# happykygo/GNN-eCommerce

Hardware: AMD Instinct MI355X
Metric: edges propagated/sec per LGConv layer (higher is better)
Workload: dtype f32; 1 GPU; configs[1]: 1639358 users x 54571 items, 20314816 directed edges, 3 LGConv layers, emb_dim 64, get_embedding (K hops + fused layer sum); parallelism=single, seed=0

## Files before the change

gnn-ecommerce_amd/_native.py:

```python
from __future__ import annotations

import ctypes
import os
from ctypes import CFUNCTYPE, POINTER, Structure, c_char_p, c_float, c_int, c_int32, c_int64, c_size_t, c_uint64, c_void_p
from typing import Optional

import torch

LIB_NAME = "liblgconv_hip.so"
LIB_PATH = os.environ.get("LGCN_LIB_PATH") or os.path.join(os.path.dirname(os.path.abspath(__file__)), "csrc", LIB_NAME)
ABI_VERSION = 14

ST_INDEX_OOB = 1
ST_SAMPLER_EXHAUSTED = 2

class SweepCfg(Structure):
    _fields_ = [("n_bands", c_int32), ("waves_per_band_round", c_int32), ("row_cap", c_int32), ("piece_cap", c_int32),
                ("lookahead", c_int32), ("groups", c_int32), ("round_order", c_int32), ("light_len", c_int32)]


class SweepDims(Structure):
    _fields_ = [("n_bands", c_int32), ("rounds", c_int32), ("row_cap", c_int32), ("piece_cap", c_int32),
                ("n_rows", c_int32), ("groups", c_int32),
                ("n_waves", c_int64), ("n_slabs", c_int64), ("n_slots", c_int64), ("n_entries", c_int64),
# ... 111 lines not shown
                              c_void_p, c_void_p, c_void_p]),
    "lgc_fold_in": (c_int, [c_void_p, c_void_p, c_void_p, c_int64, c_void_p, c_void_p, c_int64, c_int64, c_void_p, c_void_p,
                            c_int64, c_int64, c_float, c_int32, c_int32, c_void_p, c_int64, c_void_p, c_void_p]),
    "lgc_score_rows": (c_int, [c_void_p, c_int64, c_int64, c_void_p, c_int64, c_void_p, c_int64, c_int32, c_int32, c_void_p,
                               c_int64, c_void_p, c_void_p]),
    "lgc_topk_hits": (c_int, [c_void_p, c_int64, c_int32, c_void_p, c_void_p, c_void_p, c_int64, c_int64, c_void_p, c_void_p,
                              c_void_p, c_void_p]),
    "lgc_metric_sums": (c_int, [c_void_p, c_void_p, c_int64, c_void_p, c_void_p, c_void_p]),
    "lgc_rank_metrics": (c_int, [c_void_p, c_int64, c_int32, c_void_p, c_void_p, c_void_p, c_void_p, c_int64, c_int64,
                                 POINTER(c_int32), c_int32, c_void_p, c_void_p, c_void_p, c_void_p, c_void_p]),
    "lgc_column_sums": (c_int, [c_void_p, c_int64, c_int64, c_int32, c_void_p, c_void_p]),
    "lgc_topk_coverage": (c_int, [c_void_p, c_int64, c_int32, c_int64, POINTER(c_int32), c_int32, c_int64, c_void_p, c_void_p,
                                  c_void_p, c_void_p]),
    "lgc_bfs_init": (c_int, [c_void_p, c_int32, c_int64, c_void_p, c_void_p, c_void_p, c_void_p]),
    "lgc_bfs_level": (c_int, [c_void_p, c_void_p, c_int32, c_int32, c_int32, c_void_p, c_int32, c_uint64, c_void_p, c_void_p,
                              c_void_p, c_void_p, c_void_p]),
    "lgc_bfs_resolve": (c_int, [c_void_p, c_void_p, c_int32, c_int64, c_int64, c_void_p, c_int32, c_void_p, c_void_p, c_void_p,
                                c_void_p]),
    "lgc_bfs_backtrack": (c_int, [c_void_p, c_void_p, c_int64, c_void_p, c_int32, c_void_p, c_void_p, c_int32, c_int64,
                                  c_void_p, c_int32, c_void_p]),
    "lgc_sample_triples": (c_int, [c_void_p, c_int64, c_void_p, c_void_p, c_void_p, c_void_p, c_int64, c_int64, c_uint64,
                                   c_uint64, c_void_p, c_void_p, c_void_p, c_void_p]),
    "lgc_pair_dot": (c_int, [c_void_p, c_int64, c_int32, c_int64, c_void_p, c_void_p, c_int64, c_void_p,
                             c_void_p, c_void_p]),
    "lgc_reduce_workspace_bytes": (c_size_t, [c_int64, c_int64]),
    "lgc_reduce_count": (c_int, [c_void_p, c_void_p, c_int64, c_int64, c_int64, c_int32, c_void_p, c_size_t, c_void_p, c_void_p,
                                 c_void_p]),
    "lgc_reduce_fill": (c_int, [c_void_p, c_void_p, c_int64, c_int64, c_int64, c_void_p, c_void_p, c_int64, c_int64, c_void_p,
                                c_void_p, c_void_p]),
    "lgc_reduce_gram_workspace_bytes": (c_size_t, [c_int64]),
    "lgc_reduce_gram_count": (c_int, [c_void_p, c_void_p, c_int64, c_int64, c_int64, c_void_p, c_int64, c_void_p, c_size_t,
                                      c_void_p, c_void_p]),
    "lgc_reduce_gram_fill": (c_int, [c_void_p, c_int64, c_int64, c_int64, c_int64, c_void_p, c_void_p, c_void_p]),
    "lgc_attribute": (c_int, [POINTER(AttrArgsC), c_void_p]),
    "lgc_row_rnorm": (c_int, [c_void_p, c_int64, c_int64, c_int32, c_void_p, c_void_p]),
    "lgc_item_neighbors_workspace_bytes": (c_size_t, [c_int64, c_int64, c_int32, c_int32]),
    "lgc_item_neighbors": (c_int, [c_void_p, c_int64, c_int64, c_int32, c_void_p, c_int64, c_void_p, c_void_p, c_int32, c_int32,
                                   c_int32, c_void_p, c_void_p, c_void_p, c_size_t, c_void_p, c_void_p]),
    "lgc_rerank_route": (c_int, [c_int32, c_int32]),
    "lgc_rerank_mmr": (c_int, [c_void_p, c_int64, c_int64, c_int32, c_void_p, c_void_p, c_int64, c_void_p, c_int64, c_int64,
                               c_int32, c_int32, c_float, c_void_p, c_void_p, c_void_p, c_void_p, c_void_p]),
    "lgc_list_diversity": (c_int, [c_void_p, c_int64, c_int64, c_int32, c_void_p, c_void_p, c_int64, c_int64, c_int32,
                                   POINTER(c_int32), c_int32, c_void_p, c_int64, c_void_p, c_void_p]),
}


class NativeLibraryError(RuntimeError):
    """The HIP library is missing, stale, or a call into it failed."""


_lib: Optional[ctypes.CDLL] = None


def load() -> ctypes.CDLL:
    global _lib
    if _lib is not None:
        return _lib
    if not os.path.isfile(LIB_PATH):
        raise NativeLibraryError(
            f"{LIB_PATH} not found: the MI355X propagation library has not been built. "
            "Run `python -c 'import __graft_entry__ as g; g.build()'` (or `make -C gnn-ecommerce_amd/csrc`). "
            "There is no CPU or PyTorch fallback for this path.")
    try:
        lib = ctypes.CDLL(LIB_PATH)
    except OSError as exc:
        raise NativeLibraryError(f"cannot load {LIB_PATH}: {exc}") from exc
# ... 71 lines not shown
```

gnn-ecommerce_amd/csrc/lgconv_reduce.hip:

```cpp
#include "lgconv_common.h"

#include <hipcub/hipcub.hpp>

namespace {

inline size_t r_align_up(size_t v, size_t a) { return (v + a - 1) / a * a; }

struct ReduceWs {
    int32_t *incount;
    int32_t *keep_scan;
    int32_t *ent_scan;
    long long *pair_scan;
    void *cub;
    size_t cub_bytes;
};

size_t reduce_ws(void *base, int64_t n_nodes, int64_t n_edges, ReduceWs *ws) {
    size_t cb32 = 0, cb64 = 0;
    int32_t *n32 = nullptr;
    long long *n64 = nullptr;
    const int64_t longest = std::max<int64_t>(n_edges, n_nodes) + 1;
    (void)hipcub::DeviceScan::ExclusiveSum(nullptr, cb32, n32, n32, (int)longest, (hipStream_t)0);
    (void)hipcub::DeviceScan::ExclusiveSum(nullptr, cb64, n64, n64, (int)longest, (hipStream_t)0);
    const size_t cb = std::max(cb32, cb64);
// ... 17 lines not shown
    unsigned long long *keys_in, *keys_out;
    double *vals_in, *vals_out;
    int32_t *head_scan;
    void *cub;
    size_t cub_bytes;
};

size_t gram_ws(void *base, int64_t n_pairs, GramWs *ws) {
    size_t cb_sort = 0, cb_scan = 0;
    unsigned long long *nk = nullptr;
    double *nv = nullptr;
    int32_t *n32 = nullptr;
    const int64_t n = std::max<int64_t>(n_pairs, 1);
    (void)hipcub::DeviceRadixSort::SortPairs(nullptr, cb_sort, nk, nk, nv, nv, (int)n, 0, 64, (hipStream_t)0);
    (void)hipcub::DeviceScan::ExclusiveSum(nullptr, cb_scan, n32, n32, (int)(n + 1), (hipStream_t)0);
    const size_t cb = std::max(cb_sort, cb_scan);
    const uintptr_t p = reinterpret_cast<uintptr_t>(base);
    size_t off = 0;
    auto take = [&](size_t bytes) { const size_t at = off; off += r_align_up(bytes, 256); return p + at; };
    const uintptr_t a_ki = take((size_t)n * 8), a_ko = take((size_t)n * 8), a_vi = take((size_t)n * 8), a_vo = take((size_t)n * 8),
                    a_hs = take((size_t)(n + 1) * 4), a_cub = take(cb);
    if (ws) {
        ws->keys_in = reinterpret_cast<unsigned long long *>(a_ki);
        ws->keys_out = reinterpret_cast<unsigned long long *>(a_ko);
        ws->vals_in = reinterpret_cast<double *>(a_vi);
        ws->vals_out = reinterpret_cast<double *>(a_vo);
        ws->head_scan = reinterpret_cast<int32_t *>(a_hs);
        ws->cub = reinterpret_cast<void *>(a_cub);
        ws->cub_bytes = cb;
    }
    return off + 256;
}

__device__ inline int32_t row_of_entry(const int32_t *__restrict__ rowptr, int32_t n_rows, int32_t e) {
    int32_t lo = 0, hi = n_rows;
    while (hi - lo > 1) {
        const int32_t mid = lo + (hi - lo) / 2;
        if (rowptr[mid] <= e) lo = mid; else hi = mid;
    }
    return lo;
}

__global__ void k_reduce_incount(const int32_t *__restrict__ rowptr, const lgc_entry *__restrict__ entries, int32_t n_nodes,
                                 int32_t split, int32_t n_edges, int32_t *__restrict__ incount) {
    const int32_t e_begin = max(rowptr[split], 0), e_end = min(rowptr[n_nodes], n_edges);
    for (int64_t e = e_begin + (int64_t)blockIdx.x * blockDim.x + threadIdx.x; e < e_end; e += (int64_t)gridDim.x * blockDim.x) {
        const int32_t c = entries[e].col;
        if (c >= 0 && c < split) atomicAdd(incount + c, 1);
    }
}

__global__ void k_reduce_keep(const int32_t *__restrict__ rowptr, const int32_t *__restrict__ incount, int32_t split,
                              int32_t max_deg, int32_t *__restrict__ keep) {
    const int64_t u = (int64_t)blockIdx.x * blockDim.x + threadIdx.x;
    if (u > split) return;
    int32_t k = 0;
    if (u < split) k = (rowptr[u + 1] - rowptr[u] <= max_deg && incount[u] <= max_deg) ? 0 : 1;
    keep[u] = k;
}

__global__ void k_reduce_user_map(const int32_t *__restrict__ keep_scan, int32_t split, int32_t *__restrict__ user_map) {
    const int64_t u = (int64_t)blockIdx.x * blockDim.x + threadIdx.x;
    if (u >= split) return;
    user_map[u] = keep_scan[u + 1] != keep_scan[u] ? keep_scan[u] : -1;
}

__global__ void k_reduce_entry_flags(const int32_t *__restrict__ rowptr, const lgc_entry *__restrict__ entries, int32_t n_nodes,
// ... 93 lines not shown
__global__ void k_gram_fill_entries(const unsigned long long *__restrict__ keys, const double *__restrict__ vals,
                                    const int32_t *__restrict__ head_scan, long long n_pairs, int32_t n_h, int32_t n_out,
                                    lgc_entry *__restrict__ out) {
    const int64_t p = (int64_t)blockIdx.x * blockDim.x + threadIdx.x;
    if (p >= n_pairs) return;
    const int32_t dst = head_scan[p];
    if (head_scan[p + 1] == dst || dst < 0 || dst >= n_out) return;
    const unsigned long long key = keys[p];
    double sum = 0.0;
    for (int64_t q = p; q < n_pairs && keys[q] == key; ++q) sum += vals[q];
    lgc_entry en;
    en.col = n_h + (int32_t)(uint32_t)(key & 0xFFFFFFFFull);
    en.val = (float)sum;
    out[dst] = en;
}

__global__ void k_gram_fill_rowptr(const unsigned long long *__restrict__ keys, const int32_t *__restrict__ head_scan,
                                   long long n_pairs, int32_t n_h, int32_t n_items, int32_t *__restrict__ rowptr_out) {
    const int64_t r = (int64_t)blockIdx.x * blockDim.x + threadIdx.x;
    if (r > (int64_t)n_h + n_items) return;
    if (r <= n_h) {
        rowptr_out[r] = 0;
        return;
    }
    const unsigned long long want = (unsigned long long)(uint32_t)(r - n_h) << 32;
    long long lo = 0, hi = n_pairs;
    while (lo < hi) {
        const long long mid = lo + (hi - lo) / 2;
        if (keys[mid] < want) lo = mid + 1; else hi = mid;
    }
    rowptr_out[r] = head_scan[lo];
}

int reduce_args_ok(const int32_t *rowptr, const lgc_entry *entries, int64_t n_nodes, int64_t n_edges, int64_t split) {
    if (n_nodes < 0 || n_edges < 0 || split < 0) return LGC_E_INVAL;
    if (n_nodes >= INT32_MAX || n_edges >= INT32_MAX) return LGC_E_RANGE;
    if (!rowptr || split <= 0 || split >= n_nodes || (n_edges > 0 && !entries)) return LGC_E_INVAL;
    return 0;
}

}

extern "C" {

size_t lgc_reduce_workspace_bytes(int64_t n_nodes, int64_t n_edges) {
    if (n_nodes < 0 || n_edges < 0 || n_nodes >= INT32_MAX || n_edges >= INT32_MAX) return 0;
    return reduce_ws(nullptr, n_nodes, n_edges, nullptr);
}

int lgc_reduce_count(const int32_t *rowptr, const lgc_entry *entries, int64_t n_nodes, int64_t n_edges, int64_t split,
                     int32_t max_deg, void *workspace, size_t workspace_bytes, int32_t *user_map, int64_t *totals,
                     void *stream_) {
    if (const int rc = reduce_args_ok(rowptr, entries, n_nodes, n_edges, split)) return rc;
    if (max_deg < 0 || !workspace || !user_map || !totals) return LGC_E_INVAL;
    if (workspace_bytes < lgc_reduce_workspace_bytes(n_nodes, n_edges)) return LGC_E_WORKSPACE;
    if (reinterpret_cast<uintptr_t>(workspace) % 256 != 0) return LGC_E_ALIGN;
    hipStream_t st = as_stream(stream_);
    ReduceWs ws;
    reduce_ws(workspace, n_nodes, n_edges, &ws);
    const int32_t n = (int32_t)n_nodes, sp = (int32_t)split;
    hipError_t err = hipMemsetAsync(ws.incount, 0, (size_t)(split + 1) * 4, st);
    if (err != hipSuccess) return (int)err;
    if (n_edges > 0)
        hipLaunchKernelGGL(k_reduce_incount, dim3((unsigned)std::min<int64_t>(ceil_div(n_edges, kBlock), 256 * 16)), dim3(kBlock), 0,
                           st, rowptr, entries, n, sp, (int32_t)n_edges, ws.incount);
    hipLaunchKernelGGL(k_reduce_keep, dim3(ceil_div(split + 1, kBlock)), dim3(kBlock), 0, st, rowptr, ws.incount, sp, max_deg,
// ... 60 lines not shown
    hipLaunchKernelGGL(k_gram_expand, dim3(ceil_div(n_edges, kBlock)), dim3(kBlock), 0, st, rowptr, entries, n, sp, ws.pair_scan,
                       (long long)n_pairs, (int32_t)n_edges, gw.keys_in, gw.vals_in);
    err = hipcub::DeviceRadixSort::SortPairs(gw.cub, gw.cub_bytes, gw.keys_in, gw.keys_out, gw.vals_in, gw.vals_out, (int)n_pairs,
                                             0, 64, st);
    if (err != hipSuccess) return (int)err;
    hipLaunchKernelGGL(k_gram_heads, dim3(ceil_div(n_pairs + 1, kBlock)), dim3(kBlock), 0, st, gw.keys_out, (long long)n_pairs,
                       gw.head_scan);
    err = hipcub::DeviceScan::ExclusiveSum(gw.cub, gw.cub_bytes, gw.head_scan, gw.head_scan, (int)(n_pairs + 1), st);
    if (err != hipSuccess) return (int)err;
    err = hipMemcpyAsync(total, gw.head_scan + n_pairs, sizeof(int32_t), hipMemcpyDeviceToDevice, st);
    if (err != hipSuccess) return (int)err;
    return (int)hipGetLastError();
}

int lgc_reduce_gram_fill(const void *gram_workspace, int64_t n_pairs, int64_t n_kept, int64_t n_items, int64_t n_out,
                         int32_t *rowptr_out, lgc_entry *entries_out, void *stream_) {
    if (n_pairs < 0 || n_kept < 0 || n_items < 1 || n_out < 0 || !rowptr_out) return LGC_E_INVAL;
    if (n_pairs >= INT32_MAX || n_kept + n_items >= INT32_MAX) return LGC_E_RANGE;
    if (n_out > n_pairs || (n_pairs > 0 && !gram_workspace) || (n_out > 0 && !entries_out)) return LGC_E_INVAL;
    if (reinterpret_cast<uintptr_t>(gram_workspace) % 256 != 0) return LGC_E_ALIGN;
    hipStream_t st = as_stream(stream_);
    const int64_t rows = n_kept + n_items;
    if (n_pairs == 0) return (int)hipMemsetAsync(rowptr_out, 0, (size_t)(rows + 1) * 4, st);
    GramWs gw;
    gram_ws(const_cast<void *>(gram_workspace), n_pairs, &gw);
    hipLaunchKernelGGL(k_gram_fill_rowptr, dim3(ceil_div(rows + 1, kBlock)), dim3(kBlock), 0, st, gw.keys_out, gw.head_scan,
                       (long long)n_pairs, (int32_t)n_kept, (int32_t)n_items, rowptr_out);
    if (n_out > 0)
        hipLaunchKernelGGL(k_gram_fill_entries, dim3(ceil_div(n_pairs, kBlock)), dim3(kBlock), 0, st, gw.keys_out, gw.vals_out,
                           gw.head_scan, (long long)n_pairs, (int32_t)n_kept, (int32_t)n_out, entries_out);
    return (int)hipGetLastError();
}

}
```

gnn-ecommerce_amd/graph.py:

```python
from __future__ import annotations

import os
from collections import OrderedDict
from dataclasses import dataclass, field
from typing import Dict, List, Optional, Tuple

import torch
from torch import Tensor

from . import _native

SHORT_MAX = int(os.environ.get("LGCN_SHORT_MAX", "32"))
CHUNK_LEN = int(os.environ.get("LGCN_CHUNK_LEN", "256"))
USER_CHUNK_LEN = int(os.environ.get("LGCN_USER_CHUNK_LEN", "4096"))
TILE_WIDTHS = (8, 16, 32)
USE_TILES = os.environ.get("LGCN_TILES", "1") == "1"
TILES_PER_WAVE = int(os.environ.get("LGCN_TILES_PER_WAVE", "1"))
TILE_ORDER = os.environ.get("LGCN_TILE_ORDER", "cold")
USE_SWEEP = os.environ.get("LGCN_SWEEP", "auto")
SWEEP_MIN_ENTRIES = int(os.environ.get("LGCN_SWEEP_MIN_ENTRIES", "1000000"))
SWEEP_ADAPTIVE_BANDS = os.environ.get("LGCN_SWEEP_ADAPTIVE_BANDS", "1") == "1"
SWEEP_PIECE_ENTRIES = int(os.environ.get("LGCN_SWEEP_PIECE_ENTRIES", "20"))
SWEEP_CFG = dict(n_bands=int(os.environ.get("LGCN_SWEEP_BANDS", "8")), waves_per_band_round=int(os.environ.get("LGCN_SWEEP_WAVES", "256")),
                 row_cap=int(os.environ.get("LGCN_SWEEP_ROW_CAP", "78")),
                 piece_cap=int(os.environ.get("LGCN_SWEEP_PIECE_CAP", "64")),
                 lookahead=int(os.environ.get("LGCN_SWEEP_LOOKAHEAD", "64")),
                 groups=4,
                 round_order=int(os.environ.get("LGCN_SWEEP_ROUND_ORDER", "2")))
SWEEP_WIDE = os.environ.get("LGCN_SWEEP_WIDE", "1") == "1"
SWEEP_LIGHT_LEN = os.environ.get("LGCN_SWEEP_LIGHT_LEN", "auto")
SWEEP_LIGHT_LEN_WIDE = os.environ.get("LGCN_SWEEP_LIGHT_LEN_WIDE", "0")


def _light_len(value: str) -> int:
    return -1 if value == "auto" else max(int(value), 0)


PLAN_TIMING = os.environ.get("LGCN_PLAN_TIMING", "0") == "1"
# ... 625 lines not shown
    i32 = dict(dtype=torch.int32, device=dev)
    ws_bytes = lib.lgc_reduce_workspace_bytes(num_nodes, n_edges)
    ws = torch.empty(max(ws_bytes, 1), **u8)
    user_map = torch.empty(max(split, 1), **i32)
    totals = torch.empty(4, dtype=torch.int64, device=dev)
    args = (_native.ptr(rowptr), _native.ptr(entries), num_nodes, n_edges, split)
    with torch.cuda.device(dev):
        st = _native.stream_of(dev)
        _native.check(lib.lgc_reduce_count(*args, int(max_deg), _native.ptr(ws), ws_bytes, _native.ptr(user_map),
                                           _native.ptr(totals), st), "lgc_reduce_count")
        n_h, user_nnz, nnz, n_pairs = totals.tolist()
        rowptr_h = torch.empty(n_h + n_items + 1, **i32)
        entries_h = torch.empty((nnz, 2), **i32)
        _native.check(lib.lgc_reduce_fill(*args, _native.ptr(ws), _native.ptr(user_map), n_h, nnz, _native.ptr(rowptr_h),
                                          _native.ptr(entries_h) if nnz else None, st), "lgc_reduce_fill")
        gws_bytes = lib.lgc_reduce_gram_workspace_bytes(n_pairs)
        if gws_bytes == 0:
            return None
        gws = torch.empty(gws_bytes, **u8)
        total = torch.empty(1, dtype=torch.int64, device=dev)
        code = lib.lgc_reduce_gram_count(*args, _native.ptr(ws), n_pairs, _native.ptr(gws), gws_bytes, _native.ptr(total), st)
        if code == -4:
            return None
        _native.check(code, "lgc_reduce_gram_count")
        gram_nnz = int(total.item())
        gram_rowptr = torch.empty(n_h + n_items + 1, **i32)
        gram_entries = torch.empty((gram_nnz, 2), **i32)
        _native.check(lib.lgc_reduce_gram_fill(_native.ptr(gws), n_pairs, n_h, n_items, gram_nnz, _native.ptr(gram_rowptr),
                                               _native.ptr(gram_entries) if gram_nnz else None, st), "lgc_reduce_gram_fill")
    return ReducedCSR(int(max_deg), n_h, n_items, user_map[:split], rowptr_h, entries_h, user_nnz, n_pairs, gram_rowptr,
                      gram_entries)


@dataclass
class ReducedGraph:
    csr: ReducedCSR
    n_h: int
    offset: int
    user_op_h: Optional[Operator]
    item_op_h: Optional[Operator]
    gram_op: Optional[Operator]

    def nbytes(self) -> int:
        c = self.csr
        total = sum(t.numel() * 4 for t in (c.user_map, c.rowptr, c.entries, c.gram_rowptr, c.gram_entries))
        for op in (self.user_op_h, self.item_op_h, self.gram_op):
            if op is not None:
                total += op.plan.chunks.numel() * 4 + sum(tc.slab.numel() * 4 + tc.order.numel() * 4 + tc.meta.numel() * 4
                                                          for tc in (op._tiles or []))
                total += sum(sw.nbytes() for sw in op._sweep.values())
        return total


def sweep_choice(lib, dim: int, table_rows: int, stride: int) -> int:
    sweep = int(lib.lgc_sweep_ok(dim, table_rows, stride))
    return 0 if (sweep == 2 and not SWEEP_WIDE) else sweep


def _check_table(t: Tensor, name: str) -> None:
    _native.require_device(t, name)
    if t.dtype != torch.float32 or t.dim() != 2 or t.stride(1) != 1:
        raise TypeError(f"{name} must be a 2-D fp32 tensor with unit inner stride, got {t.dtype} {tuple(t.shape)}")


class PropGraph:

    def __init__(self, edge_index: Tensor, edge_weight: Optional[Tensor], num_nodes: int,
                 normalize: bool = True, short_max: int = SHORT_MAX, chunk_len: int = CHUNK_LEN,
                 keep_edge_values: bool = False):
        _native.require_device(edge_index, "edge_index")
        if edge_index.dtype != torch.int64 or edge_index.dim() != 2 or edge_index.size(0) != 2:
            raise TypeError("edge_index must be an int64 tensor of shape [2, E]")
        if edge_weight is not None:
            _native.require_device(edge_weight, "edge_weight")
            if edge_weight.dtype != torch.float32 or edge_weight.shape != (edge_index.size(1),):
                raise TypeError("edge_weight must be fp32 of shape [E]")
            if edge_weight.device != edge_index.device:
                raise RuntimeError("edge_index and edge_weight must be on the same device")
        self.device = edge_index.device
# ... 73 lines not shown
        auto = forced is None and ELIMINATE_MAX_DEG == "auto"
        max_deg = int(forced) if forced is not None else (ELIMINATE_AUTO_MAX_DEG if auto else int(ELIMINATE_MAX_DEG))
        if max_deg <= 0:
            return None
        key = ("reduced", max_deg, auto)
        if key in self._halves:
            return self._halves[key]
        got = None
        if not auto or self.halves(False)[1].sweep_cols is not None:
            got = self._build_reduced(max_deg)
            if got is not None and auto:
                removed = self.forward_op.nnz - got.csr.nnz
                if got.csr.gram_nnz > ELIMINATE_MAX_GRAM_SHARE * removed:
                    got = None
        self._halves[key] = got
        return got

    def _build_reduced(self, max_deg: int) -> Optional[ReducedGraph]:
        op = self.forward_op
        csr = build_reduced_csr(op.rowptr, op.entries, self.split, self.num_nodes, max_deg)
        if csr is None:
            return None
        n_h, n_rows = csr.n_h, csr.n_h + csr.n_items
        user_chunk = max(self.chunk_len, USER_CHUNK_LEN)
        user_op_h = item_op_h = gram_op = None
        if n_h > 0:
            user_op_h = Operator.build(n_rows, csr.rowptr, csr.entries, 0, n_h, self.short_max, user_chunk,
                                       sweep_cols=(n_h, n_rows))
        if csr.nnz - csr.user_nnz > 0:
            item_op_h = Operator.build(n_rows, csr.rowptr, csr.entries, n_h, n_rows, self.short_max, self.chunk_len,
                                       sweep_cols=(0, n_h))
        if csr.gram_nnz > 0:
            gram_op = Operator.build(n_rows, csr.gram_rowptr, csr.gram_entries, n_h, n_rows, self.short_max, GRAM_CHUNK_LEN)
        return ReducedGraph(csr, n_h, self.split - n_h, user_op_h, item_op_h, gram_op)

    def prepare(self, dim: int, table_rows: Optional[int] = None, transpose: bool = False) -> "PropGraph":
        lib = _native.load()
        rows = self.num_nodes if table_rows is None else int(table_rows)
        stride = dim if dim % 32 == 0 else (dim + 31) // 32 * 32
        ops = self.halves(transpose) if self.split is not None else ((self.transpose_op if transpose else self.forward_op),)
        ops = [(op, rows) for op in ops]
        red = self.reduced(transpose)
        if red is not None:
            ops += [(op, max(rows - red.offset, 0)) for op in (red.user_op_h, red.item_op_h, red.gram_op) if op is not None]
        import time
        for op, rows in ops:
            t0 = time.perf_counter()
            if op.tiled and dim >= 4:
                op.tiles
            if PLAN_TIMING:
                torch.cuda.synchronize(self.device)
                print(f"[plan] rows [{op.plan.row_begin}, {op.plan.row_end}): tile classes {time.perf_counter() - t0:.3f} s", flush=True)
            t0 = time.perf_counter()
            if op.sweep_cols is not None:
                groups = sweep_choice(lib, dim, rows, stride)
                if groups:
                    op.sweep_plan(groups)
            if PLAN_TIMING:
                torch.cuda.synchronize(self.device)
                print(f"[plan] rows [{op.plan.row_begin}, {op.plan.row_end}): sweep plan total {time.perf_counter() - t0:.3f} s", flush=True)
        torch.cuda.synchronize(self.device)
        return self

    @property
    def transpose_op(self) -> Operator:
        if self._transpose_op is None:
            if self._edge_index is None:
                raise _native.NativeLibraryError("this graph was loaded from a file without its COO: the transposed "
                                                 "operator (backward pass) needs a graph built from edge_index")
            self._transpose_op = self._build(by_source=True)
        return self._transpose_op

    def save(self, path: str, extra: Optional[Dict[str, Tensor]] = None, meta: Optional[Dict[str, str]] = None) -> None:
        from safetensors.torch import save_file
        op = self.forward_op
        tensors = {"rowptr": op.rowptr, "entries": op.entries, "deg": self.deg, "dis": self.dis}
        for k, v in (extra or {}).items():
# ... 113 lines not shown
```

gnn-ecommerce_amd/propagate.py:

```python
from __future__ import annotations

import os
from typing import List, Optional, Sequence

import torch
from torch import Tensor
from torch.autograd.function import once_differentiable

from . import _native
from .graph import Operator, PropGraph, apply_rows


HOP_EVENT_LOG: Optional[list] = None


def _timed_apply(op: Operator, x: Tensor, out: Tensor, **kw) -> None:
    if HOP_EVENT_LOG is None:
        op.apply(x, out, **kw)
        return
    start, end = torch.cuda.Event(enable_timing=True), torch.cuda.Event(enable_timing=True)
    start.record()
    op.apply(x, out, **kw)
    end.record()
    HOP_EVENT_LOG.append((start, end))
# ... 23 lines not shown
        h = nxt
    return h


USE_BIPARTITE = os.environ.get("LGCN_BIPARTITE", "1") == "1"

class _HopSpan:

    def __enter__(self):
        self.log = HOP_EVENT_LOG
        if self.log is not None:
            self.start, self.end = torch.cuda.Event(enable_timing=True), torch.cuda.Event(enable_timing=True)
            self.start.record()
        return self

    def __exit__(self, *exc):
        if self.log is not None:
            self.end.record()
            self.log.append((self.start, self.end))


def bipartite_sum(user_op: Operator, item_op: Operator, split: int, x0: Tensor, alphas: Sequence[float],
                  final_rows: Optional[Tensor] = None, reduced=None) -> Tensor:
    k = len(alphas) - 1
    if k == 0:
        return x0 * alphas[0]
    x0 = x0.contiguous()
    n = x0.size(0)
    tables = [x0]
    red = reduced if k >= 2 else None
    rows_items_only = final_rows is not None and SCORED_ITEM_ROWS_ONLY and item_op.listed_rows_pay(final_rows.numel()) \
        if red is not None else False

    def user_step(layer: int, x: Tensor, out_t: Tensor) -> None:
        if red is None or (rows_items_only and layer == k - 1):
            user_op.apply(x, out_t)
        elif red.user_op_h is not None:
            red.user_op_h.apply(x[red.offset:], out_t[red.offset:])

    def item_step(layer: int, out_t: Tensor, a: float = 1.0, r: Optional[Tensor] = None) -> None:
        o = red.offset
        y = out_t[o:]
        have = r is not None
        if red.gram_op is not None:
            red.gram_op.apply(tables[layer - 2][o:], y, a=a, r=r[o:] if have else None, b=1.0 if have else 0.0)
        elif have:
            _native.lincomb(out_t[split:], [(1.0, r[split:])])
        else:
            out_t[split:].zero_()
        if red.item_op_h is not None:
            red.item_op_h.apply(tables[layer - 1][o:], y, a=a, r=y, b=1.0)
    uniform = UNIFORM_ALPHA_SHORTCUT and all(a == alphas[0] for a in alphas) and (UNIFORM_ALPHA_SHORTCUT == "force" or x0.size(1) % 32 == 0)
    for layer in range(1, k + 1):
        with _HopSpan():
            nxt = scratch_table(x0)
            if layer < k:
                if red is None or layer == 1:
                    item_op.apply(tables[-1], nxt)
                else:
                    item_step(layer, nxt)
                user_step(layer, tables[-1], nxt)
                tables.append(nxt)
            else:
                out = torch.empty_like(x0)
                rows_only = final_rows is not None
                if rows_only and SCORED_ITEM_ROWS_ONLY and item_op.listed_rows_pay(final_rows.numel()):
                    mix = nxt
                    _native.lincomb(mix[split:], [(alphas[l], tables[l - 1][split:]) for l in range(1, k + 1)])
                    if all(a == alphas[0] for a in alphas):
                        rest = mix
                    else:
                        rest = scratch_table(x0)
                        _native.lincomb(rest[split:], [(alphas[l], tables[l][split:]) for l in range(0, k)])
# ... 1083 lines not shown
```

include/lgconv_hip.h:

```cpp
#ifndef LGCONV_HIP_H
#define LGCONV_HIP_H

#include <stddef.h>
#include <stdint.h>

#ifdef __cplusplus
extern "C" {
#endif

#define LGC_ABI_VERSION 14

#define LGC_E_INVAL      (-1)
#define LGC_E_DIM        (-2)
#define LGC_E_WORKSPACE  (-3)
#define LGC_E_RANGE      (-4)
#define LGC_E_ALIGN      (-5)

#define LGC_ST_INDEX_OOB 1

typedef struct lgc_entry {
    int32_t col;
    float   val;
} lgc_entry;

// ... 250 lines not shown
#define LGC_BFS_UNSET (-3)
int lgc_bfs_init(const int64_t *sources, int32_t n_sources, int64_t n_nodes, uint64_t *seen, uint64_t *frontier,
                 int32_t *status, void *stream);
int lgc_bfs_level(const int32_t *rowptr, const lgc_entry *entries, int32_t row_begin, int32_t row_end, int32_t short_max,
                  const lgc_chunk *chunks, int32_t n_chunks, uint64_t active, const uint64_t *frontier_in,
                  uint64_t *frontier_out, uint64_t *seen, uint64_t *counters, void *stream);
int lgc_bfs_resolve(const int64_t *sources, const int64_t *targets, int32_t n_sources, int64_t n_targets, int64_t n_nodes,
                    const uint64_t *frontier, int32_t level, int32_t *dist, uint64_t *counters, int32_t *status,
                    void *stream);
int lgc_bfs_backtrack(const int32_t *rowptr, const lgc_entry *entries, int64_t n_nodes, const uint64_t *levels,
                      int32_t n_levels, const int64_t *targets, const int32_t *dist, int32_t n_sources, int64_t n_targets,
                      int64_t *paths, int32_t path_len, void *stream);

#define LGC_ST_SAMPLER_EXHAUSTED 2
int lgc_sample_triples(const int64_t *users, int64_t n,
                       const int32_t *pos_ptr, const int64_t *pos_items,
                       const int32_t *ign_ptr, const int64_t *ign_items,
                       int64_t n_users, int64_t n_items, uint64_t seed, uint64_t step,
                       int64_t *pos_out, int64_t *neg_out, int32_t *status, void *stream);

size_t lgc_reduce_workspace_bytes(int64_t n_nodes, int64_t n_edges);
int lgc_reduce_count(const int32_t *rowptr, const lgc_entry *entries, int64_t n_nodes, int64_t n_edges, int64_t split,
                     int32_t max_deg, void *workspace, size_t workspace_bytes, int32_t *user_map, int64_t *totals,
                     void *stream);
int lgc_reduce_fill(const int32_t *rowptr, const lgc_entry *entries, int64_t n_nodes, int64_t n_edges, int64_t split,
                    const void *workspace, const int32_t *user_map, int64_t n_kept, int64_t n_out, int32_t *rowptr_out,
                    lgc_entry *entries_out, void *stream);
size_t lgc_reduce_gram_workspace_bytes(int64_t n_pairs);
int lgc_reduce_gram_count(const int32_t *rowptr, const lgc_entry *entries, int64_t n_nodes, int64_t n_edges, int64_t split,
                          const void *workspace, int64_t n_pairs, void *gram_workspace, size_t gram_workspace_bytes,
                          int64_t *total, void *stream);
int lgc_reduce_gram_fill(const void *gram_workspace, int64_t n_pairs, int64_t n_kept, int64_t n_items, int64_t n_out,
                         int32_t *rowptr_out, lgc_entry *entries_out, void *stream);

#define LGC_ATTR_MAX_TARGETS 64
#define LGC_ATTR_MAX_TOP 8
typedef struct lgc_attr_args {
    const int64_t   *list_ptr, *list_items;
    const float     *list_weight, *item_dis;
    const int32_t   *rowptr;
    const lgc_entry *entries;
    const int64_t   *row_ids;
    int64_t          n_graph_rows, col_base;
    int64_t          n_rows;
    const float     *fold, *items;
    int64_t          fold_stride, item_stride, n_items;
    const int64_t   *init_rows;
    const float     *init;
    int64_t          init_stride, n_init_rows;
    const int64_t   *targets;
    int64_t          target_stride;
    const int64_t   *contrib_ptr;
    float           *contrib, *base, *total;
    int32_t         *top_pos;
    int64_t         *top_item;
    float           *top_value;
    int32_t         *status;
    float            a0;
    int32_t          normalize, n_targets, top_m, dim;
} lgc_attr_args;

int lgc_attribute(const lgc_attr_args *args, void *stream);

#define LGC_NEIGHBORS_MAX_K 64
int lgc_row_rnorm(const float *table, int64_t stride, int64_t n_rows, int32_t dim, float *out, void *stream);
size_t lgc_item_neighbors_workspace_bytes(int64_t n_queries, int64_t n_items, int32_t k, int32_t slices);
// ... 22 lines not shown
```

Baseline: 40.61 billion edges/s.

## Concatenate reduced user graph and item gram into one banded CSR operator

Builds a combined CSR in which the kept-user rows, an identity block stored in gap rows interleaved between user bands, the item-to-user edges and the item gram entries all live in one matrix. The item step then becomes a single sweep operator call instead of separate gram and item operators with an intermediate write. This removes one pass over the output table per layer and one kernel launch. In exchange it adds padded gap rows and a larger entry array, extra build time, and complex index arithmetic in the layout whose correctness depends on the band mapping matching the sweep configuration.

```diff
diff --git a/gnn-ecommerce_amd/_native.py b/gnn-ecommerce_amd/_native.py
--- a/gnn-ecommerce_amd/_native.py
+++ b/gnn-ecommerce_amd/_native.py
@@ -167,6 +167,11 @@
     "lgc_reduce_gram_count": (c_int, [c_void_p, c_void_p, c_int64, c_int64, c_int64, c_void_p, c_int64, c_void_p, c_size_t,
                                       c_void_p, c_void_p]),
     "lgc_reduce_gram_fill": (c_int, [c_void_p, c_int64, c_int64, c_int64, c_int64, c_void_p, c_void_p, c_void_p]),
+    "lgc_reduce_concat_rows": (c_int64, [c_int64, c_int64, c_int32]),
+    "lgc_reduce_concat": (c_int, [c_void_p, c_void_p, c_int64, c_void_p, c_void_p, c_int64, c_int64, c_int64, c_int32, c_void_p,
+                                  c_void_p, c_void_p, c_void_p, c_int64, c_void_p]),
+    "lgc_reduce_concat_host": (c_int, [c_void_p, c_void_p, c_int64, c_void_p, c_void_p, c_int64, c_int64, c_int64, c_int32,
+                                       c_void_p, c_void_p, c_void_p, c_void_p, c_int64]),
     "lgc_attribute": (c_int, [POINTER(AttrArgsC), c_void_p]),
     "lgc_row_rnorm": (c_int, [c_void_p, c_int64, c_int64, c_int32, c_void_p, c_void_p]),
     "lgc_item_neighbors_workspace_bytes": (c_size_t, [c_int64, c_int64, c_int32, c_int32]),
diff --git a/gnn-ecommerce_amd/csrc/lgconv_reduce.hip b/gnn-ecommerce_amd/csrc/lgconv_reduce.hip
--- a/gnn-ecommerce_amd/csrc/lgconv_reduce.hip
+++ b/gnn-ecommerce_amd/csrc/lgconv_reduce.hip
@@ -73,7 +73,7 @@
     return off + 256;
 }
 
-__device__ inline int32_t row_of_entry(const int32_t *__restrict__ rowptr, int32_t n_rows, int32_t e) {
+__host__ __device__ inline int32_t row_of_entry(const int32_t *__restrict__ rowptr, int32_t n_rows, int32_t e) {
     int32_t lo = 0, hi = n_rows;
     while (hi - lo > 1) {
         const int32_t mid = lo + (hi - lo) / 2;
@@ -233,6 +233,126 @@
     rowptr_out[r] = head_scan[lo];
 }
 
+struct Concat {
+    const int32_t *rp;
+    const lgc_entry *ent;
+    const int32_t *grp;
+    const lgc_entry *gent;
+    int32_t n_kept, n_items, n_gaps, gap_rows, n_phys, n_gram, n_out;
+    int32_t *pos, *gap_start, *rowptr_out;
+    lgc_entry *out;
+};
+
+__host__ __device__ inline int32_t cc_band(const Concat &c, int32_t h) {
+    const int64_t ne = c.rp[c.n_kept];
+    if (ne <= 0) return 0;
+    const int64_t b = (int64_t)c.rp[h] * c.n_gaps / ne;
+    return (int32_t)(b < c.n_gaps - 1 ? b : c.n_gaps - 1);
+}
+
+__host__ __device__ inline int32_t cc_users_upto(const Concat &c, int32_t b) {
+    const int64_t ne = c.rp[c.n_kept];
+    if (b >= c.n_gaps - 1 || ne <= 0) return c.n_kept;
+    int32_t lo = 0, hi = c.n_kept;
+    while (lo < hi) {
+        const int32_t mid = lo + (hi - lo) / 2;
+        if ((int64_t)c.rp[mid] * c.n_gaps < ne * (b + 1)) lo = mid + 1; else hi = mid;
+    }
+    return lo;
+}
+
+__host__ __device__ inline int32_t cc_min(int64_t a, int64_t b) { return (int32_t)(a < b ? a : b); }
+
+__host__ __device__ inline void cc_layout_at(const Concat &c, int64_t t) {
+    if (t < c.n_kept) c.pos[t] = (int32_t)t + c.gap_rows * cc_band(c, (int32_t)t);
+    else if (t < (int64_t)c.n_kept + c.n_gaps) {
+        const int32_t b = (int32_t)(t - c.n_kept);
+        c.gap_start[b] = cc_users_upto(c, b) + c.gap_rows * b;
+    }
+}
+
+__host__ __device__ inline void cc_rowptr_at(const Concat &c, int64_t r) {
+    if (r > (int64_t)c.n_phys + c.n_items) return;
+    int64_t v;
+    if (r >= c.n_phys) {
+        const int32_t i = (int32_t)(r - c.n_phys);
+        v = (int64_t)c.rp[c.n_kept] + c.n_items + (c.rp[c.n_kept + i] - c.rp[c.n_kept]) + c.grp[c.n_kept + i];
+    } else {
+        int32_t before = 0;
+        while (before < c.n_gaps && c.gap_start[before] <= r) ++before;
+        if (before > 0 && r < (int64_t)c.gap_start[before - 1] + c.gap_rows) {
+            const int32_t b = before - 1;
+            const int64_t j = (int64_t)b * c.gap_rows + (r - c.gap_start[b]);
+            v = (int64_t)c.rp[c.gap_start[b] - c.gap_rows * b] + cc_min(j, c.n_items);
+        } else {
+            const int32_t h = (int32_t)(r - (int64_t)c.gap_rows * before);
+            v = (int64_t)c.rp[h] + cc_min((int64_t)before * c.gap_rows, c.n_items);
+        }
+    }
+    c.rowptr_out[r] = (int32_t)v;
+}
+
+__host__ __device__ inline void cc_entry_at(const Concat &c, int64_t t) {
+    const int64_t n_user = c.rp[c.n_kept], n_all = c.rp[c.n_kept + c.n_items];
+    const int64_t first_item_entry = n_user + c.n_items;
+    int64_t dst;
+    lgc_entry en;
+    if (t < n_user) {
+        const int32_t h = row_of_entry(c.rp, c.n_kept, (int32_t)t);
+        en = c.ent[t];
+        en.col = c.n_phys + (en.col - c.n_kept);
+        dst = t + cc_min((int64_t)cc_band(c, h) * c.gap_rows, c.n_items);
+    } else if ((t -= n_user) < c.n_items) {
+        const int32_t b = (int32_t)(t / c.gap_rows);
+        en.col = c.n_phys + (int32_t)t;
+        en.val = 1.0f;
+        dst = (int64_t)c.rp[c.gap_start[b] - c.gap_rows * b] + t;
+    } else if ((t -= c.n_items) < n_all - n_user) {
+        const int64_t e = n_user + t;
+        const int32_t i = row_of_entry(c.rp + c.n_kept, c.n_items, (int32_t)e);
+        en = c.ent[e];
+        en.col = c.pos[en.col];
+        dst = first_item_entry + t + c.grp[c.n_kept + i];
+    } else if ((t -= n_all - n_user) < c.n_gram) {
+        const int32_t i = row_of_entry(c.grp + c.n_kept, c.n_items, (int32_t)t);
+        en = c.gent[t];
+        const int32_t j = en.col - c.n_kept;
+        en.col = c.gap_start[j / c.gap_rows] + j % c.gap_rows;
+        dst = first_item_entry + (c.rp[c.n_kept + i + 1] - n_user) + t;
+    } else {
+        return;
+    }
+    if (dst >= 0 && dst < c.n_out) c.out[dst] = en;
+}
+
+__global__ void k_concat_layout(Concat c) {
+    const int64_t t = (int64_t)blockIdx.x * blockDim.x + threadIdx.x;
+    cc_layout_at(c, t);
+}
+__global__ void k_concat_rowptr(Concat c) {
+    const int64_t r = (int64_t)blockIdx.x * blockDim.x + threadIdx.x;
+    cc_rowptr_at(c, r);
+}
+__global__ void k_concat_entries(Concat c) {
+    const int64_t t = (int64_t)blockIdx.x * blockDim.x + threadIdx.x;
+    if (t < c.n_out) cc_entry_at(c, t);
+}
+
+int concat_args(const int32_t *rowptr, const lgc_entry *entries, int64_t n_entries, const int32_t *gram_rowptr,
+                const lgc_entry *gram_entries, int64_t n_gram, int64_t n_kept, int64_t n_items, int32_t n_gaps,
+                int32_t *user_pos, int32_t *gap_start, int32_t *rowptr_out, lgc_entry *entries_out, int64_t n_out, Concat *c) {
+    if (n_entries < 0 || n_gram < 0 || n_kept < 0 || n_items < 1 || n_gaps < 1 || n_out < 0) return LGC_E_INVAL;
+    if (n_gaps > LGC_REDUCE_MAX_GAPS) return LGC_E_RANGE;
+    const int64_t gap_rows = (n_items + n_gaps - 1) / n_gaps, n_phys = n_kept + gap_rows * n_gaps;
+    if (n_phys + n_items >= INT32_MAX || n_entries + n_items + n_gram >= INT32_MAX) return LGC_E_RANGE;
+    if (!rowptr || !gram_rowptr || !gap_start || !rowptr_out || !entries_out || (n_entries > 0 && !entries) ||
+        (n_gram > 0 && !gram_entries) || (n_kept > 0 && !user_pos) || n_out != n_entries + n_items + n_gram)
+        return LGC_E_INVAL;
+    *c = Concat{rowptr, entries, gram_rowptr, gram_entries, (int32_t)n_kept, (int32_t)n_items, n_gaps, (int32_t)gap_rows,
+                (int32_t)n_phys, (int32_t)n_gram, (int32_t)n_out, user_pos, gap_start, rowptr_out, entries_out};
+    return 0;
+}
+
 int reduce_args_ok(const int32_t *rowptr, const lgc_entry *entries, int64_t n_nodes, int64_t n_edges, int64_t split) {
     if (n_nodes < 0 || n_edges < 0 || split < 0) return LGC_E_INVAL;
     if (n_nodes >= INT32_MAX || n_edges >= INT32_MAX) return LGC_E_RANGE;
@@ -359,4 +479,38 @@
     return (int)hipGetLastError();
 }
 
-}
+int64_t lgc_reduce_concat_rows(int64_t n_kept, int64_t n_items, int32_t n_gaps) {
+    if (n_kept < 0 || n_items < 1 || n_gaps < 1 || n_gaps > LGC_REDUCE_MAX_GAPS) return -1;
+    return n_kept + (n_items + n_gaps - 1) / n_gaps * n_gaps;
+}
+
+int lgc_reduce_concat(const int32_t *rowptr, const lgc_entry *entries, int64_t n_entries, const int32_t *gram_rowptr,
+                      const lgc_entry *gram_entries, int64_t n_gram, int64_t n_kept, int64_t n_items, int32_t n_gaps,
+                      int32_t *user_pos, int32_t *gap_start, int32_t *rowptr_out, lgc_entry *entries_out, int64_t n_out,
+                      void *stream_) {
+    Concat c;
+    if (const int rc = concat_args(rowptr, entries, n_entries, gram_rowptr, gram_entries, n_gram, n_kept, n_items, n_gaps,
+                                   user_pos, gap_start, rowptr_out, entries_out, n_out, &c))
+        return rc;
+    hipStream_t st = as_stream(stream_);
+    hipLaunchKernelGGL(k_concat_layout, dim3(ceil_div(n_kept + n_gaps, kBlock)), dim3(kBlock), 0, st, c);
+    hipLaunchKernelGGL(k_concat_rowptr, dim3(ceil_div((int64_t)c.n_phys + n_items + 1, kBlock)), dim3(kBlock), 0, st, c);
+    hipLaunchKernelGGL(k_concat_entries, dim3(ceil_div(n_out, kBlock)), dim3(kBlock), 0, st, c);
+    return (int)hipGetLastError();
+}
+
+int lgc_reduce_concat_host(const int32_t *rowptr, const lgc_entry *entries, int64_t n_entries, const int32_t *gram_rowptr,
+                           const lgc_entry *gram_entries, int64_t n_gram, int64_t n_kept, int64_t n_items, int32_t n_gaps,
+                           int32_t *user_pos, int32_t *gap_start, int32_t *rowptr_out, lgc_entry *entries_out, int64_t n_out) {
+    Concat c;
+    if (const int rc = concat_args(rowptr, entries, n_entries, gram_rowptr, gram_entries, n_gram, n_kept, n_items, n_gaps,
+                                   user_pos, gap_start, rowptr_out, entries_out, n_out, &c))
+        return rc;
+    if (rowptr[n_kept + n_items] != n_entries || gram_rowptr[n_kept + n_items] != n_gram) return LGC_E_INVAL;
+    for (int64_t t = 0; t < n_kept + n_gaps; ++t) cc_layout_at(c, t);
+    for (int64_t r = 0; r <= (int64_t)c.n_phys + n_items; ++r) cc_rowptr_at(c, r);
+    for (int64_t t = 0; t < n_out; ++t) cc_entry_at(c, t);
+    return 0;
+}
+
+}
diff --git a/gnn-ecommerce_amd/graph.py b/gnn-ecommerce_amd/graph.py
--- a/gnn-ecommerce_amd/graph.py
+++ b/gnn-ecommerce_amd/graph.py
@@ -3,7 +3,7 @@
 import os
 from collections import OrderedDict
 from dataclasses import dataclass, field
-from typing import Dict, List, Optional, Tuple
+from typing import Callable, Dict, List, Optional, Tuple
 
 import torch
 from torch import Tensor
@@ -695,6 +695,53 @@
                       gram_entries)
 
 
+REDUCED_CONCAT = os.environ.get("LGCN_REDUCED_CONCAT", "auto")
+if REDUCED_CONCAT not in ("0", "1", "auto"):
+    raise ValueError(f"LGCN_REDUCED_CONCAT must be 0, 1 or auto, got {REDUCED_CONCAT!r}")
+
+
+@dataclass
+class ConcatCSR:
+    n_gaps: int
+    gap_rows: int
+    n_phys: int
+    user_pos: Tensor
+    gap_start: Tensor
+    rowptr: Tensor
+    entries: Tensor
+
+
+def build_concat_csr(csr: ReducedCSR, n_gaps: int, host: bool = False) -> ConcatCSR:
+    lib = _native.load()
+    dev = csr.rowptr.device
+    if not host:
+        _native.require_device(csr.rowptr, "rowptr")
+    n_phys = int(lib.lgc_reduce_concat_rows(csr.n_h, csr.n_items, n_gaps))
+    if n_phys < 0:
+        raise ValueError(f"no concatenated layout for {csr.n_h} kept users, {csr.n_items} items and {n_gaps} gaps")
+    i32 = dict(dtype=torch.int32, device=dev)
+    n_out = csr.nnz + csr.n_items + csr.gram_nnz
+    user_pos, gap_start = torch.empty(max(csr.n_h, 1), **i32), torch.empty(n_gaps, **i32)
+    rowptr, entries = torch.empty(n_phys + csr.n_items + 1, **i32), torch.empty((n_out, 2), **i32)
+    args = (_native.ptr(csr.rowptr), _native.ptr(csr.entries) if csr.nnz else None, csr.nnz, _native.ptr(csr.gram_rowptr),
+            _native.ptr(csr.gram_entries) if csr.gram_nnz else None, csr.gram_nnz, csr.n_h, csr.n_items, n_gaps,
+            _native.ptr(user_pos), _native.ptr(gap_start), _native.ptr(rowptr), _native.ptr(entries), n_out)
+    if host:
+        _native.check(lib.lgc_reduce_concat_host(*args), "lgc_reduce_concat_host")
+    else:
+        with torch.cuda.device(dev):
+            _native.check(lib.lgc_reduce_concat(*args, _native.stream_of(dev)), "lgc_reduce_concat")
+    return ConcatCSR(n_gaps, (csr.n_items + n_gaps - 1) // n_gaps, n_phys, user_pos[:csr.n_h], gap_start, rowptr, entries)
+
+
+@dataclass
+class ConcatGraph:
+    csr: ConcatCSR
+    offset: int
+    user_op: Operator
+    item_op: Operator
+
+
 @dataclass
 class ReducedGraph:
     csr: ReducedCSR
@@ -703,11 +750,32 @@
     user_op_h: Optional[Operator]
     item_op_h: Optional[Operator]
     gram_op: Optional[Operator]
+    concat_build: Optional[Callable[[], Optional[ConcatGraph]]] = None
+    concat_mode: Optional[str] = None
+    _concat: Optional[list] = None
+
+    def concat_for(self, dim: int, table_rows: int, stride: int) -> Optional[ConcatGraph]:
+        mode = self.concat_mode if self.concat_mode is not None else REDUCED_CONCAT
+        if mode == "0" or self.concat_build is None or self.gram_op is None:
+            return None
+        if mode == "auto" and (self.item_op_h is None or self.item_op_h.sweep_cols is None):
+            return None
+        if self._concat is None:
+            self._concat = [self.concat_build()]
+        cc = self._concat[0]
+        if cc is None or mode == "1":
+            return cc
+        if cc.item_op.sweep_cols is None:
+            return None
+        return cc if sweep_choice(_native.load(), dim, max(table_rows - cc.offset, 0), stride) else None
 
     def nbytes(self) -> int:
         c = self.csr
         total = sum(t.numel() * 4 for t in (c.user_map, c.rowptr, c.entries, c.gram_rowptr, c.gram_entries))
-        for op in (self.user_op_h, self.item_op_h, self.gram_op):
+        cc = self._concat[0] if self._concat else None
+        if cc is not None:
+            total += sum(t.numel() * 4 for t in (cc.csr.user_pos, cc.csr.gap_start, cc.csr.rowptr, cc.csr.entries))
+        for op in (self.user_op_h, self.item_op_h, self.gram_op) + ((cc.user_op, cc.item_op) if cc is not None else ()):
             if op is not None:
                 total += op.plan.chunks.numel() * 4 + sum(tc.slab.numel() * 4 + tc.order.numel() * 4 + tc.meta.numel() * 4
                                                           for tc in (op._tiles or []))
@@ -847,7 +915,20 @@
                                        sweep_cols=(0, n_h))
         if csr.gram_nnz > 0:
             gram_op = Operator.build(n_rows, csr.gram_rowptr, csr.gram_entries, n_h, n_rows, self.short_max, GRAM_CHUNK_LEN)
-        return ReducedGraph(csr, n_h, self.split - n_h, user_op_h, item_op_h, gram_op)
+
+        def concat() -> Optional[ConcatGraph]:
+            n_gaps = int(SWEEP_CFG["n_bands"])
+            n_phys = int(_native.load().lgc_reduce_concat_rows(n_h, csr.n_items, n_gaps))
+            if csr.gram_nnz == 0 or n_phys < 0 or n_phys > self.split:
+                return None
+            cc = build_concat_csr(csr, n_gaps)
+            rows = n_phys + csr.n_items
+            return ConcatGraph(cc, self.split - n_phys,
+                               Operator.build(rows, cc.rowptr, cc.entries, 0, n_phys, self.short_max, user_chunk,
+                                              sweep_cols=(n_phys, rows)),
+                               Operator.build(rows, cc.rowptr, cc.entries, n_phys, rows, self.short_max, self.chunk_len,
+                                              sweep_cols=(0, n_phys)))
+        return ReducedGraph(csr, n_h, self.split - n_h, user_op_h, item_op_h, gram_op, concat_build=concat)
 
     def prepare(self, dim: int, table_rows: Optional[int] = None, transpose: bool = False) -> "PropGraph":
         lib = _native.load()
@@ -857,7 +938,11 @@
         ops = [(op, rows) for op in ops]
         red = self.reduced(transpose)
         if red is not None:
-            ops += [(op, max(rows - red.offset, 0)) for op in (red.user_op_h, red.item_op_h, red.gram_op) if op is not None]
+            cc = red.concat_for(dim, rows, stride)
+            if cc is not None:
+                ops += [(cc.user_op, max(rows - cc.offset, 0)), (cc.item_op, max(rows - cc.offset, 0))]
+            else:
+                ops += [(op, max(rows - red.offset, 0)) for op in (red.user_op_h, red.item_op_h, red.gram_op) if op is not None]
         import time
         for op, rows in ops:
             t0 = time.perf_counter()
diff --git a/gnn-ecommerce_amd/propagate.py b/gnn-ecommerce_amd/propagate.py
--- a/gnn-ecommerce_amd/propagate.py
+++ b/gnn-ecommerce_amd/propagate.py
@@ -79,13 +79,22 @@
     rows_items_only = final_rows is not None and SCORED_ITEM_ROWS_ONLY and item_op.listed_rows_pay(final_rows.numel()) \
         if red is not None else False
 
+    cc = red.concat_for(x0.size(1), n, x0.size(1) if (not PAD_INTERNAL or x0.size(1) % 32 == 0)
+                        else (x0.size(1) + 31) // 32 * 32) if red is not None else None
+
     def user_step(layer: int, x: Tensor, out_t: Tensor) -> None:
         if red is None or (rows_items_only and layer == k - 1):
             user_op.apply(x, out_t)
+        elif cc is not None:
+            cc.user_op.apply(x[cc.offset:], out_t[cc.offset:])
         elif red.user_op_h is not None:
             red.user_op_h.apply(x[red.offset:], out_t[red.offset:])
 
     def item_step(layer: int, out_t: Tensor, a: float = 1.0, r: Optional[Tensor] = None) -> None:
+        if cc is not None:
+            o = cc.offset
+            cc.item_op.apply(tables[layer - 1][o:], out_t[o:], a=a, r=None if r is None else r[o:], b=0.0 if r is None else 1.0)
+            return
         o = red.offset
         y = out_t[o:]
         have = r is not None
diff --git a/include/lgconv_hip.h b/include/lgconv_hip.h
--- a/include/lgconv_hip.h
+++ b/include/lgconv_hip.h
@@ -306,6 +306,16 @@
                           int64_t *total, void *stream);
 int lgc_reduce_gram_fill(const void *gram_workspace, int64_t n_pairs, int64_t n_kept, int64_t n_items, int64_t n_out,
                          int32_t *rowptr_out, lgc_entry *entries_out, void *stream);
+
+#define LGC_REDUCE_MAX_GAPS 64
+int64_t lgc_reduce_concat_rows(int64_t n_kept, int64_t n_items, int32_t n_gaps);
+int lgc_reduce_concat(const int32_t *rowptr, const lgc_entry *entries, int64_t n_entries, const int32_t *gram_rowptr,
+                      const lgc_entry *gram_entries, int64_t n_gram, int64_t n_kept, int64_t n_items, int32_t n_gaps,
+                      int32_t *user_pos, int32_t *gap_start, int32_t *rowptr_out, lgc_entry *entries_out, int64_t n_out,
+                      void *stream);
+int lgc_reduce_concat_host(const int32_t *rowptr, const lgc_entry *entries, int64_t n_entries, const int32_t *gram_rowptr,
+                           const lgc_entry *gram_entries, int64_t n_gram, int64_t n_kept, int64_t n_items, int32_t n_gaps,
+                           int32_t *user_pos, int32_t *gap_start, int32_t *rowptr_out, lgc_entry *entries_out, int64_t n_out);
 
 #define LGC_ATTR_MAX_TARGETS 64
 #define LGC_ATTR_MAX_TOP 8
```

Result: faster. 41.39 billion edges/s, median of 6 (+1.9%).
